# google-research/tnco

Hardware: AMD Instinct MI355X
Metric: SA move-evaluations/s (whole node) + best log10(flops) vs ref, 512-leaf TN (higher is better)
Workload: dtype f64

## Files before the change

tnco_amd/csrc/sa_kernels.h:

```cpp
#pragma once
#include <hip/hip_runtime.h>
#include <stdint.h>

namespace tnco {

#ifndef TNCO_LPS
#define TNCO_LPS 1
#endif
constexpr int LPS = TNCO_LPS;

struct __attribute__((aligned(32))) NodeRec {
  int32_t left, right, parent, pad;
  union { double ccost; double pleft; };
  union { double partial; double pright; };
};
struct __attribute__((aligned(16))) Links {
  int32_t left, right, parent, pad;
};
struct __attribute__((aligned(128))) ReplicaState {
  double min_cost;
  double init_total;
  unsigned long long n_moves, n_accepted, n_improved;
  int32_t mti;
  int32_t mtw;
  int32_t status;
  int32_t jinvalid;
  unsigned long long n_randpick;
  uint32_t jmin, jtail;
  double total;
  unsigned long long n_fullcopy;
  unsigned long long pad1[5];
};
static_assert(sizeof(NodeRec) == 32, "NodeRec");
static_assert(sizeof(ReplicaState) == 128, "ReplicaState");

struct Params {
  int32_t n, N, I, W;
  int32_t BS;
  int32_t WS;
  int32_t WOFF;
  int64_t RB;
  int32_t jcap;
  int64_t R;
  uint8_t* blocks;
  int32_t* lpar;
  uint32_t* mt;
  uint32_t* mtshadow;
  ReplicaState* rs;
  Links* minlinks;
  int32_t* jlog;
  const uint64_t* leafmask;
  const uint64_t* outmask;
  int32_t cost_mode;
  int32_t log2d;
  const double* ctab;
  const double* dimsd;
  const uint64_t* oddmask;
  int32_t odd_single;
  const uint64_t* sparse;
  double n_projs;
  int32_t f32;
  int32_t disable_shared;
  const uint64_t* dimclass;
  int32_t n_dimclass;
  int32_t cpl;
};

template <int K>
struct Mask {
  uint64_t w[K];
};
template <int K>
__device__ __forceinline__ Mask<K> mzero() {
  Mask<K> r;
#pragma unroll
  for (int k = 0; k < K; ++k) r.w[k] = 0;
  return r;
}
#define TNCO_MASK_OP(NAME, EXPR)                                                  \
  template <int K>                                                                \
  __device__ __forceinline__ Mask<K> NAME(const Mask<K>& a, const Mask<K>& b) {   \
    Mask<K> r;                                                                    \
    _Pragma("unroll") for (int k = 0; k < K; ++k) r.w[k] = (EXPR);                \
    return r;                                                                     \
  }
TNCO_MASK_OP(mand, a.w[k] & b.w[k])
TNCO_MASK_OP(mor, a.w[k] | b.w[k])
TNCO_MASK_OP(mxor, a.w[k] ^ b.w[k])
TNCO_MASK_OP(mandn, a.w[k] & ~b.w[k])
#undef TNCO_MASK_OP
template <int K>
__device__ __forceinline__ uint32_t mpopc(const Mask<K>& a) {
  uint32_t c = 0;
#pragma unroll
  for (int k = 0; k < K; ++k) c += (uint32_t)__popcll(a.w[k]);
  return c;
}
template <int K>
__device__ __forceinline__ bool mnonzero(const Mask<K>& a) {
  uint64_t x = 0;
#pragma unroll
  for (int k = 0; k < K; ++k) x |= a.w[k];
  return x != 0;
}
template <int K>
__device__ __forceinline__ bool mdiffer(const Mask<K>& a, const Mask<K>& b) {
  return mnonzero<K>(mxor<K>(a, b));
}
template <int K>
__device__ __forceinline__ Mask<K> msel(bool c, const Mask<K>& a, const Mask<K>& b) {
  Mask<K> r;
#pragma unroll
  for (int k = 0; k < K; ++k) r.w[k] = c ? a.w[k] : b.w[k];
  return r;
}

typedef uint64_t u64x2 __attribute__((ext_vector_type(2)));
typedef uint32_t u32x2 __attribute__((ext_vector_type(2)));
template <int K>
struct PairStage {
  u64x2 p[K / 2 ? K / 2 : 1];
  uint64_t s;
};
template <int LOG2L, int K, bool HYPER, bool UNI = false, bool PAIRS = false>
struct View {
  static constexpr int L = 1 << LOG2L;
  static constexpr int LK = L * K;
  static constexpr int KP = K / 2;
  uint8_t* blk;
  int32_t* lpar;
  const uint64_t* leafmask;
  uint64_t* hyp;
  int n, BS, W, lig, WS, WOFF;

  __device__ __forceinline__ void init(const Params& P, uint8_t* blk_, int32_t* lpar_, int lig_, uint64_t* hyp_ = nullptr) {
    blk = blk_; lpar = lpar_; leafmask = P.leafmask; n = P.n; BS = P.BS; W = P.W; lig = lig_;
    WS = P.WS; WOFF = P.WOFF; hyp = hyp_;
  }
  __device__ __forceinline__ NodeRec* hdr(int p) const {
    return reinterpret_cast<NodeRec*>(blk + (int64_t)(p - n) * BS);
  }
  __device__ __forceinline__ uint32_t hdr_piece_off(int p) const { return (uint32_t)(p - n) * (uint32_t)BS + 8u * (uint32_t)(lig & 3); }
  __device__ __forceinline__ int widx(int k) const {
    if constexpr (PAIRS) return k < 2 * KP ? 2 * L * (k >> 1) + 2 * lig + (k & 1) : 2 * L * KP + lig;
    return k * L + lig;
  }
  __device__ __forceinline__ uint64_t* words(int p) const {
    if constexpr (UNI) return reinterpret_cast<uint64_t*>(blk + (int64_t)(p - n) * BS + 32);
    return reinterpret_cast<uint64_t*>(blk + WOFF + (int64_t)(p - n) * WS);
  }
  __device__ __forceinline__ uint64_t* hwords(int p) const { return hyp + (int64_t)(p - n) * W; }
  __device__ __forceinline__ Mask<K> mask(int x) const {
    const bool leaf = x < n;
    const uint64_t* s = leaf ? leafmask + (int64_t)x * LK : words(x);
    Mask<K> r;
#pragma unroll
    for (int k = 0; k < K; ++k) {
      const int i = widx(k);
      r.w[k] = s[(leaf || i < W) ? i : W - 1];
    }
#pragma unroll
    for (int k = 0; k < K; ++k)
      if (!leaf && widx(k) >= W) r.w[k] = 0ull;
    return r;
  }
  __device__ __forceinline__ Mask<K> mask_staged(int x) const {
    const bool leaf = x < n;
    const uint64_t* s = leaf ? leafmask + (int64_t)x * LK : words(x);
    Mask<K> r;
#pragma unroll
    for (int k = 0; k < K; ++k) {
      r.w[k] = 0ull;
      if (leaf || widx(k) < W) r.w[k] = s[widx(k)];
    }
    return r;
  }
  __device__ __forceinline__ void mask_stage_into(Mask<K>& r, int x) const {
    const bool leaf = x < n;
    const uint64_t* s = leaf ? leafmask + (int64_t)x * LK : words(x);
#pragma unroll
    for (int k = 0; k < K; ++k)
      if (leaf || widx(k) < W) r.w[k] = s[widx(k)];
  }
  __device__ __forceinline__ void set_mask(int p, const Mask<K>& v) const {
    uint64_t* s = words(p);
#pragma unroll
    for (int k = 0; k < K; ++k)
      if (widx(k) < W) s[widx(k)] = v.w[k];
  }
  __device__ __forceinline__ void pair_stage_into(PairStage<K>& g, int x) const {
    const bool leaf = x < n;
    const uint64_t* s = leaf ? leafmask + (int64_t)x * LK : words(x);
#pragma unroll
    for (int j = 0; j < KP; ++j)
      if (leaf || widx(2 * j) < W) g.p[j] = *reinterpret_cast<const u64x2*>(s + widx(2 * j));
    if constexpr (K & 1)
      if (leaf || widx(K - 1) < W) g.s = s[widx(K - 1)];
  }
  __device__ __forceinline__ Mask<K> pair_landed(PairStage<K>& g) const {
    Mask<K> r;
#pragma unroll
    for (int j = 0; j < KP; ++j) {
      if (widx(2 * j + 1) >= W) g.p[j].y = 0ull;
      r.w[2 * j] = g.p[j].x;
      r.w[2 * j + 1] = g.p[j].y;
    }
    if constexpr (K & 1) r.w[K - 1] = g.s;
    return r;
  }
  __device__ __forceinline__ void set_mask_pairs(int p, const Mask<K>& v) const {
    uint64_t* s = words(p);
#pragma unroll
    for (int j = 0; j < KP; ++j)
      if (widx(2 * j) < W) {
        u64x2 t;
        t.x = v.w[2 * j]; t.y = v.w[2 * j + 1];
        *reinterpret_cast<u64x2*>(s + widx(2 * j)) = t;
      }
    if constexpr (K & 1)
      if (widx(K - 1) < W) s[widx(K - 1)] = v.w[K - 1];
  }
  __device__ __forceinline__ void set_mask_first(int p, const Mask<K>& v) const {
    if (widx(0) < W) words(p)[widx(0)] = v.w[0];
  }
  __device__ __forceinline__ Mask<K> hyper(int p) const {
    Mask<K> r = mzero<K>();
    if constexpr (HYPER) {
      const uint64_t* s = hwords(p);
#pragma unroll
      for (int k = 0; k < K; ++k)
        if (widx(k) < W) r.w[k] = s[widx(k)];
    }
    return r;
  }
  __device__ __forceinline__ void set_hyper(int p, const Mask<K>& v) const {
    if constexpr (HYPER) {
      if (hyp == nullptr) return;
      uint64_t* s = hwords(p);
#pragma unroll
      for (int k = 0; k < K; ++k)
        if (widx(k) < W) s[widx(k)] = v.w[k];
    }
  }
  __device__ __forceinline__ double partial(int x) const {
    const double* a = x < n ? reinterpret_cast<const double*>(leafmask) : &hdr(x)->partial;
    const double p = *a;
    return x < n ? 0.0 : p;
  }
  __device__ __forceinline__ int parent(int x) const {
    const int32_t* a = x < n ? lpar + (int64_t)x * LPS : &hdr(x)->parent;
    return *a;
  }
  __device__ __forceinline__ void set_parent(int x, int p) const {
    if (x < n) lpar[(int64_t)x * LPS] = p; else hdr(x)->parent = p;
  }
  __device__ __forceinline__ void set_parent_group(int x, int p) const {
    if (x < n) {
      if constexpr (LPS == 16) {
        if (lig < 4) *reinterpret_cast<int4*>(lpar + (int64_t)x * LPS + 4 * lig) = make_int4(p, p, p, p);
      } else {
        if (lig == 0) lpar[(int64_t)x * LPS] = p;
      }
    } else if (lig == 0) {
      hdr(x)->parent = p;
    }
  }
  __device__ __forceinline__ void set_parent_lane0(int x, int p) const {
    int32_t* a = x < n ? lpar + (int64_t)x * LPS : &hdr(x)->parent;
    if (lig == 0) *a = p;
  }
  __device__ __forceinline__ int left(int x) const { return x < n ? -1 : hdr(x)->left; }
  __device__ __forceinline__ int right(int x) const { return x < n ? -1 : hdr(x)->right; }
};

__device__ inline int cpl_cost_exp(const Params& P, const uint8_t* blk, int lk, int l, int rr) {
  auto legs = [&](int x) -> const uint64_t* {
    return x < P.n ? P.leafmask + (int64_t)x * lk : reinterpret_cast<const uint64_t*>(blk + (int64_t)(x - P.n) * P.BS + 32);
  };
  const uint64_t *a = legs(l), *b = legs(rr);
  int pc = 0;
  for (int w = 0; w < P.W; ++w) pc += __popcll(a[w] | b[w]);
  return P.log2d * pc;
}
__device__ inline double cpl_partial(const Params& P, const uint8_t* blk, int64_t r, int p, int parent) {
  if (parent < 0) return P.rs[r].total;
  const NodeRec* h = reinterpret_cast<const NodeRec*>(blk + (int64_t)(parent - P.n) * P.BS);
  return h->left == p ? h->pleft : h->pright;
}

#define TNCO_DPP_XOR1 0xB1
#define TNCO_DPP_XOR2 0x4E
#define TNCO_DPP_HALF_MIRROR 0x141
#define TNCO_DPP_MIRROR 0x140

template <int CTRL>
__device__ __forceinline__ uint32_t dpp(uint32_t v) {
  return (uint32_t)__builtin_amdgcn_update_dpp(0, (int)v, CTRL, 0xF, 0xF, false);
}

template <int J>
__device__ __forceinline__ uint32_t quad_bcast(uint32_t v) {
  return dpp<J * 0x55>(v);
}

template <int LOG2L>
__device__ __forceinline__ uint32_t gsum(uint32_t v) {
  if constexpr (LOG2L >= 1) v += dpp<TNCO_DPP_XOR1>(v);
  if constexpr (LOG2L >= 2) v += dpp<TNCO_DPP_XOR2>(v);
  if constexpr (LOG2L >= 3) v += dpp<TNCO_DPP_HALF_MIRROR>(v);
  if constexpr (LOG2L >= 4) v += dpp<TNCO_DPP_MIRROR>(v);
  if constexpr (LOG2L >= 5) v += (uint32_t)__shfl_xor((int)v, 16);
  if constexpr (LOG2L >= 6) v += (uint32_t)__shfl_xor((int)v, 32);
  return v;
}

template <int LOG2L>
__device__ __forceinline__ uint32_t gmax(uint32_t v) {
  auto mx = [](uint32_t a, uint32_t b) { return a > b ? a : b; };
  if constexpr (LOG2L >= 1) v = mx(v, dpp<TNCO_DPP_XOR1>(v));
  if constexpr (LOG2L >= 2) v = mx(v, dpp<TNCO_DPP_XOR2>(v));
  if constexpr (LOG2L >= 3) v = mx(v, dpp<TNCO_DPP_HALF_MIRROR>(v));
  if constexpr (LOG2L >= 4) v = mx(v, dpp<TNCO_DPP_MIRROR>(v));
  if constexpr (LOG2L >= 5) v = mx(v, (uint32_t)__shfl_xor((int)v, 16));
  if constexpr (LOG2L >= 6) v = mx(v, (uint32_t)__shfl_xor((int)v, 32));
  return v;
}

template <int LOG2L>
__device__ __forceinline__ bool gany(bool p) {
  return gsum<LOG2L>(p ? 1u : 0u) != 0u;
}

__device__ __forceinline__ double rnd_cost(double x, int f32) {
  return f32 ? (double)(float)x : x;
}

__device__ __forceinline__ double pow2_cost(int e, int f32) {
  double v = (e > 1023) ? __builtin_huge_val() : __hiloint2double((1023 + e) << 20, 0);
  return f32 ? (double)(float)v : v;
}

typedef __attribute__((address_space(3))) const double lds_cdouble;

template <int LOG2L>
__device__ __forceinline__ uint64_t group_bcast(uint64_t x, int j, int gbase) {
  uint32_t lo = (uint32_t)x, hi = (uint32_t)(x >> 32);
  if constexpr (LOG2L <= 2) {
    uint32_t l2, h2;
    switch (j) {
      case 0: l2 = dpp<0x00>(lo); h2 = dpp<0x00>(hi); break;
      case 1: l2 = dpp<0x55>(lo); h2 = dpp<0x55>(hi); break;
      case 2: l2 = dpp<0xAA>(lo); h2 = dpp<0xAA>(hi); break;
// ... 393 lines not shown
```

tnco_amd/csrc/sa_sweep.h:

```cpp
#pragma once
#include "sa_kernels.h"
#include "fw_params.h"

#include <type_traits>

namespace tnco {

#define TNCO_LANDED(x) __asm__ volatile("" : "+v"(x) : : "memory")

#ifndef TNCO_NODE_ACCESS
#define TNCO_NODE_ACCESS 4
#endif

#define TNCO_LDS __attribute__((address_space(3)))
typedef TNCO_LDS volatile uint32_t lds_vu32;
typedef TNCO_LDS volatile int32_t lds_vi32;

__device__ __forceinline__ uint32_t mt_temper(uint32_t z) {
  z ^= (z >> 11);
  z ^= (z << 7) & 0x9d2c5680u;
  z ^= (z << 15) & 0xefc60000u;
  z ^= (z >> 18);
  return z;
}

constexpr int MT_SHADOW = 64;

constexpr int MT_ROUND_RING = 64;
constexpr int MT_ROUND_LOW = 8;
static_assert(MT_ROUND_RING <= MT_SHADOW && MT_ROUND_LOW >= 7, "refill rounds");

typedef uint32_t rng_u32x4 __attribute__((ext_vector_type(4)));
struct RngPcv { rng_u32x4 pcv; };
struct RngNoPcv {};
template <int LOG2L, int RINGX = 0, bool PCV = false>
struct Rng : std::conditional_t<PCV, RngPcv, RngNoPcv> {
  static constexpr int L = 1 << LOG2L;
  static constexpr int NL = L < 4 ? L : 4;
  static constexpr int SB = 4 * NL;
  static constexpr int RING = RINGX ? RINGX : ((2 * SB > 16) ? 2 * SB : 16);
  static_assert(RING <= MT_SHADOW && (RING & (RING - 1)) == 0 && RING >= 2 * SB, "ring size");

  struct __attribute__((packed, aligned(4))) U4 { uint32_t x[4]; };

  uint32_t* mt_base;
  uint32_t* sh_base;
  uint32_t r32;
  lds_vu32* ring;
  int lig;
  __device__ __forceinline__ uint32_t* st() const { return mt_base + (uint64_t)r32 * 624u; }
  __device__ __forceinline__ uint32_t* shadow() const { return sh_base + (uint64_t)r32 * (uint32_t)MT_SHADOW; }
  uint32_t cons, prod, tw;
  bool pend, ptw;
  typedef rng_u32x4 u32x4;
  u32x4 pa;
  uint32_t pb, pc[4];
  typedef u32x4 u32x4w __attribute__((aligned(4)));

  __device__ __forceinline__ uint32_t gen_of_cons() const { return cons == 0 ? 0u : (cons - 1u) / 624u; }

  __device__ __forceinline__ void request() {
    const uint32_t k0 = prod % 624u;
    ptw = prod >= tw;
    if (lig < NL) {
      const int k = (int)k0 + 4 * lig;
      const uint32_t* s = st();
      pa = *reinterpret_cast<const u32x4*>(s + k);
      if (ptw) {
        pb = s[(k + 4 == 624) ? 0 : k + 4];
        if (k == 224) {
          if constexpr (PCV) { this->pcv.x = s[621]; this->pcv.y = s[622]; this->pcv.z = s[623]; this->pcv.w = s[0]; }
          else { pc[0] = s[621]; pc[1] = s[622]; pc[2] = s[623]; pc[3] = s[0]; }
        } else {
          int km = k + 397;
          if (km >= 624) km -= 624;
          if constexpr (PCV) {
            this->pcv = *reinterpret_cast<const u32x4w*>(s + km);
          } else {
            const U4 c = *reinterpret_cast<const U4*>(s + km);
            pc[0] = c.x[0]; pc[1] = c.x[1]; pc[2] = c.x[2]; pc[3] = c.x[3];
          }
        }
      }
    }
    pend = true;
  }
  __device__ __forceinline__ void produce() {
    if (lig < NL) {
      const uint32_t nx[4] = {pa[1], pa[2], pa[3], pb};
      uint32_t v[4];
#pragma unroll
      for (int j = 0; j < 4; ++j) {
        v[j] = pa[j];
        if (ptw) {
// ... 144 lines not shown
  } while (0)
#define TNCO_PROF_OUT(rs) \
  for (int k_ = 0; k_ < 5; ++k_) (rs)->pad1[k_] += pa_[k_]
#else
#define TNCO_PROF_DECL
#define TNCO_PROF_T(i)
#define TNCO_PROF_F(i)
#define TNCO_PROF_ACC
#define TNCO_PROF_OUT(rs)
#endif

#ifndef TNCO_SWEEP_THREADS
#define TNCO_SWEEP_THREADS 256
#endif
constexpr int SWT = TNCO_SWEEP_THREADS;
#ifndef TNCO_FW_STAGED_WAVES
#define TNCO_FW_STAGED_WAVES 2
#endif
#ifndef TNCO_LEAN_RULE
#define TNCO_LEAN_RULE (FW && !GENERIC && !HYPER && LOG2L == 2)
#endif
template <int LOG2L, int K, bool HYPER, bool GENERIC, bool FW = false, bool SPREAD = false>
#ifndef TNCO_HYPER_WAVES
#define TNCO_HYPER_WAVES 2
#endif
#ifndef TNCO_GENERIC_WAVES
#define TNCO_GENERIC_WAVES 2
#endif
#ifndef TNCO_K4_WAVES
#define TNCO_K4_WAVES 2
#endif
__device__ __forceinline__ void sa_run_body(
    const Params& P, const double* __restrict__ betas, const int64_t n_steps, const int prob_kind,
    const FwParams& F, const int tail_last, const int block0) {
  constexpr int L = 1 << LOG2L;
  constexpr int GPB = SWT >> LOG2L;
  using M = Mask<K>;
  constexpr bool ROUNDS = !HYPER && !GENERIC && !FW;
  constexpr bool RPCV = ROUNDS && TNCO_NODE_ACCESS >= 4;
  using R = Rng<LOG2L, ROUNDS ? MT_ROUND_RING : 0, RPCV>;
  static_assert(!ROUNDS || R::SB + 1 >= MT_ROUND_LOW, "refill rounds: the prologue");
  __shared__ uint32_t rngbuf[GPB * R::RING];
  __shared__ ColdState coldbuf[GPB];
  __shared__ int32_t jbuf[GPB * 16];
  constexpr bool LEAN = TNCO_LEAN_RULE;
  __shared__ WalkScal scalbuf[LEAN ? GPB : 1];
  __shared__ uint64_t slbuf[LEAN && FW ? GPB * L * K : 1];
  __shared__ double tabbuf[GENERIC ? (L * K * 64 + 1) : 1];
  __shared__ uint64_t clsbuf[GENERIC ? (TABS_MAXCLS * L * K) : 1];
  __shared__ uint64_t oddbuf[GENERIC ? (L * K) : 1];
  if constexpr (GENERIC) {
    const bool use_ctab = P.cost_mode == 1 || (P.cost_mode == 2 && P.odd_single);
    if (use_ctab) {
      for (int i = threadIdx.x; i < P.W * 64 + 1; i += SWT) tabbuf[i] = P.ctab[i];
    } else if (P.cost_mode == 2) {
      for (int i = threadIdx.x; i < L * K * 64; i += SWT) tabbuf[i] = P.dimsd[i];
    }
    if (P.cost_mode >= 2) {
      for (int i = threadIdx.x; i < P.n_dimclass * L * K; i += SWT) clsbuf[i] = P.dimclass[i];
      if (P.cost_mode == 2)
        for (int i = threadIdx.x; i < L * K; i += SWT) oddbuf[i] = P.oddmask[i];
    }
    __syncthreads();
  }

  const int tid = threadIdx.x;
  const int lig = tid & (L - 1);
  const int gbase = (tid & 63) & ~(L - 1);
  const int seats = SPREAD ? block0 : (64 >> LOG2L);
  const int gw = (tid & 63) >> LOG2L;
  const bool master = !SPREAD || gw < seats;
  const int seat = SPREAD ? (gw & (seats - 1)) : gw;
  const int gib = SPREAD ? (tid >> 6) * (64 >> LOG2L) + seat : tid >> LOG2L;
  const int64_t r = SPREAD ? ((int64_t)blockIdx.x * (SWT / 64) + (tid >> 6)) * seats + seat
                           : ((int64_t)blockIdx.x + block0) * GPB + gib;
  if (r >= P.R || n_steps <= 0) return;
  const bool lane0 = (lig == 0) && master;
  const int slig = master ? lig : (1 << 20);

  const int n = P.n, N = P.N;
  constexpr bool HYD = HYPER;
  constexpr bool CP = !HYPER && !GENERIC && !FW;
  constexpr bool QHDR = CP && TNCO_NODE_ACCESS >= 1, PAIRS = CP && TNCO_NODE_ACCESS >= 2, PSEL = CP && TNCO_NODE_ACCESS >= 3 && LPS == 1;
  View<LOG2L, K, HYPER, !FW, PAIRS> v;
  v.init(P, P.blocks + r * P.RB, nullptr, lig);
  auto lpar = [&]() -> int32_t* { return P.lpar + r * (int64_t)n * LPS; };
  lds_cold& cold = *((lds_cold*)coldbuf + gib);

  R rng;
  {
    const ReplicaState* rs = P.rs + r;
    rng.template init<ROUNDS ? 2 : 0>(P, r, (lds_vu32*)rngbuf + gib * R::RING, rs->mti, rs->mtw, master ? lig : 64);
    if (lane0) {
      cold.min_cost = rs->min_cost;
      cold.jmin = rs->jmin;
      cold.n_impr = 0; cold.n_full = 0; cold.n_rpick = 0;
    }
  }
  const uint32_t jcap = (uint32_t)P.jcap;
  uint32_t jtail = P.rs[r].jtail;
  bool jinvalid = P.rs[r].jinvalid != 0;
  auto jb = [&](int i) -> lds_vi32& { return *((lds_vi32*)jbuf + gib * 16 + i); };
  auto jlog = [&]() -> int32_t* {
    uint32_t rr = rng.r32;
    __asm__ volatile("" : "+v"(rr));
    return P.jlog + (int64_t)rr * (int64_t)P.jcap;
  };
  if ((jtail & 15u) != 0u) {
    for (int q = slig; q < 4; q += L) {
      const int4 t = *reinterpret_cast<const int4*>(jlog() + (jtail & ~15u) + 4 * q);
      jb(4 * q + 0) = t.x; jb(4 * q + 1) = t.y; jb(4 * q + 2) = t.z; jb(4 * q + 3) = t.w;
    }
  }
  M sl_regs = mzero<K>();
  typedef TNCO_LDS volatile uint64_t lds_vu64;
  [[maybe_unused]] lds_vu64* slw = (lds_vu64*)slbuf + (LEAN && FW ? gib * (L * K) : 0);
  [[maybe_unused]] bool impr_any = false;
  if constexpr (FW) {
    const uint64_t* s0 = F.slices + r * 2 * (int64_t)(L * K);
#pragma unroll
    for (int k = 0; k < K; ++k) {
      if constexpr (LEAN && FW) slw[v.widx(k)] = s0[v.widx(k)]; else sl_regs.w[k] = s0[v.widx(k)];
    }
  }
  [[maybe_unused]] TabsLds<K> tabs{P, (lds_cdouble*)tabbuf, (lds_cu64*)clsbuf, (lds_cu64*)oddbuf, mzero<K>()};
  if constexpr (GENERIC) {
    if (P.sparse != nullptr) {
#pragma unroll
      for (int k = 0; k < K; ++k) tabs.sp.w[k] = P.sparse[k * L + lig];
    }
  }
  const int f32 = GENERIC ? P.f32 : 0;
  const int log2d = P.log2d;
  const bool disable_shared = P.disable_shared != 0;
  const int nsteps32 = (int)n_steps;

  int B = 0, bl = 0, br = 0, A = -1;
  [[maybe_unused]] int wB = 0;
  double ccB = 0, partB = 0;
  WalkScal scal_regs{0, 0, 0, 0, 0, 0, 0, -1, -1, -1, -1, -1, -1, 0, 0, 0, 0};
  TNCO_LDS volatile WalkScal* scal_lds = (TNCO_LDS volatile WalkScal*)scalbuf + (LEAN ? gib : 0);
  auto& S = *[&]() {
    if constexpr (LEAN) return scal_lds; else return &scal_regs;
  }();
  if constexpr (CP) {
    double t0 = P.rs[r].total;
    TNCO_LANDED(t0);
    S.total = t0;
  }
  if constexpr (LEAN) {
    S.total = 0; S.beta = 0; S.pP = 0; S.pO = 0; S.pC = 0; S.raC = 0; S.rnC = 0;
    S.raL = -1; S.raR = -1; S.raP = -1; S.rnL = -1; S.rnR = -1; S.rnP = -1; S.raW = 0; S.rnW = 0; S.n_moves = 0; S.n_acc = 0;
  }
  M mP = mzero<K>(), mO = mzero<K>(), hB = mzero<K>();
  bool pl = true;
  M mC = mzero<K>(), hA = mzero<K>();
  int step = 0;
  int state = S_BEGIN;

  int stC = 0, stE = 0;
  [[maybe_unused]] double stW64 = 0;
  [[maybe_unused]] double stQ0 = 0, stQ1 = 0;
  int x_al = 0, x_ar = 0, x_aP = -1;
  double x_ccA = 0, x_partA = 0, x_pCcur = 0;
  int gL = -1, gR = -1, gP = -1;
  [[maybe_unused]] int gW = 0;
  double gC = 0;
  [[maybe_unused]] double gQ1 = 0;
  typedef int32_t i32x4 __attribute__((ext_vector_type(4)));
  [[maybe_unused]] i32x4 gLRP = (i32x4)(-1);
  [[maybe_unused]] u32x2 gHq = (u32x2)(0u);
  M gM = mzero<K>(), gH = mzero<K>();
  [[maybe_unused]] PairStage<K> gMq;
  if constexpr (PAIRS) {
#pragma unroll
    for (int j = 0; j < (K / 2 ? K / 2 : 1); ++j) gMq.p[j] = (u64x2)(0ull);
    gMq.s = 0ull;
  }
  uint32_t gXlo = 0, gXhi = 0;

  TNCO_PROF_DECL;
  for (;;) {
    TNCO_PROF_T(0);
    if (rng.pend) rng.produce();
    TNCO_PROF_T(1);

    bool acc = false, did_move = false, did_end = false, improved = false;

    if (state == S_END) {
      did_end = true;
      const bool close_sweep = !FW || tail_last != 0 || step != nsteps32 - 1;
      if constexpr (CP) {
        stQ0 = pl ? S.pP : S.pO;
        stQ1 = pl ? S.pO : S.pP;
      }
      if (close_sweep && partB < cold.min_cost) {
        if constexpr (FW) impr_any = true;
        if (lane0) {
          cold.min_cost = partB;
          cold.n_impr = cold.n_impr + 1;
        }
        if (jinvalid) {
          if (lane0) {
            NodeRec o;
            o.left = bl; o.right = br; o.parent = -1; o.pad = 0; o.ccost = CP ? stQ0 : ccB; o.partial = CP ? stQ1 : partB;
            *v.hdr(B) = o;
          }
          v.lpar = lpar();
          Links* __restrict__ ml = P.minlinks + r * (int64_t)N;
          for (int i0 = slig; i0 < N; i0 += 4 * L) {
            int4 h4[4];
#pragma unroll
            for (int q = 0; q < 4; ++q) {
              const int i = i0 + q * L;
              h4[q] = make_int4(-1, -1, -1, 0);
              if (i < n) h4[q].z = v.lpar[(int64_t)i * LPS];
              else if (i < N) h4[q] = *reinterpret_cast<const int4*>(v.hdr(i));
            }
#pragma unroll
            for (int q = 0; q < 4; ++q) {
              const int i = i0 + q * L;
              if (i < N) {
                Links o;
                o.left = h4[q].x; o.right = h4[q].y; o.parent = h4[q].z; o.pad = 0;
                ml[i] = o;
              }
            }
          }
          jtail = 0;
          jinvalid = false;
          if (lane0) cold.n_full = cold.n_full + 1;
        }
        improved = true;
      }
      if constexpr (CP) S.total = partB;
      ++step;
      state = (step >= nsteps32) ? -1 : S_BEGIN;
    }

    TNCO_PROF_F(1);
    int hN = -1, x1 = -1, yN = -1;
    const uint32_t* xa = nullptr;
    if (state == S_BEGIN) {
      const uint32_t x = rng.next();
      x_al = (int)(x % (uint32_t)n);
      x1 = x_al;
      xa = reinterpret_cast<const uint32_t*>(lpar() + (int64_t)x_al * LPS);
    } else if (state == S_GOT_B) {
      hN = B;
      if constexpr (CP) x1 = B;
      else xa = reinterpret_cast<const uint32_t*>(&v.hdr(B)->partial);
    } else if (CP && state == S_GOT_HB) {
      xa = reinterpret_cast<const uint32_t*>(betas + step);
      if (A >= 0) {
        hN = A;
        x1 = A;
      }
    } else if (state == S_GOT_HB) {
      x1 = pl ? br : bl;
      hN = A;
      yN = B;
      xa = reinterpret_cast<const uint32_t*>(&v.hdr(N - 1)->partial);
    } else if (state == S_GOT_B1) {
      xa = reinterpret_cast<const uint32_t*>(betas + step);
      if (A >= 0) {
        hN = S.raP;
        yN = A;
        x1 = (S.raL == B) ? S.raR : S.raL;
      }
    } else if (state == S_MOVE) {
      if constexpr (CP) {
        if (S.raP >= 0) {
          hN = S.raP;
          x1 = S.raP;
        }
      } else if (S.raP >= 0) {
        x1 = (S.rnL == A) ? S.rnR : S.rnL;
        hN = S.rnP;
        yN = S.raP;
      }
    }

    TNCO_PROF_F(2);
    if constexpr (QHDR) {
      int lq = lig;
      __asm__ volatile("" : "+v"(lq));
      v.lig = lq;
    }
    if (hN >= 0) {
      const NodeRec* q = v.hdr(hN);
      if constexpr (QHDR) {
        gHq = *reinterpret_cast<const u32x2*>(v.blk + v.hdr_piece_off(hN));
      } else {
        if constexpr (CP) gLRP = *reinterpret_cast<const i32x4*>(q);
        else { gL = q->left; gR = q->right; gP = q->parent; }
        gC = q->ccost;
        if constexpr (FW) gW = q->pad;
        if constexpr (CP) gQ1 = q->pright;
      }
    }
    double gMp = 0;
    if (x1 >= 0) {
      if constexpr (PAIRS) v.pair_stage_into(gMq, x1);
      else v.mask_stage_into(gM, x1);
      if constexpr (!CP)
        if (x1 >= n) gMp = v.hdr(x1)->partial;
    }
    if (xa != nullptr) {
      gXlo = xa[0];
      gXhi = xa[1];
    }
    if constexpr (HYPER) {
      if (yN >= 0) v.mask_stage_into(gH, yN);
    }
    if constexpr (ROUNDS) {
      const bool need = !rng.pend && rng.avail() < (uint32_t)MT_ROUND_LOW;
      const bool round = __ballot(need) != 0;
      if (round && rng.room()) rng.request();
    } else {
      if (rng.room()) rng.request();
    }
    TNCO_PROF_F(3);

    if (state == S_MOVE) {
      did_move = true;
      int al = S.raL, ar = S.raR;
      const int aP = S.raP;
      double ccA = S.raC;
      const bool c_is_right = (al == B);
      const int C = c_is_right ? ar : al;

      const M hy = HYD ? mand<K>(hB, mor<K>(mand<K>(hA, mC), mand<K>(mP, mO))) : mzero<K>();
      M sl = sl_regs;
      if constexpr (LEAN && FW) {
#pragma unroll
        for (int k = 0; k < K; ++k) sl.w[k] = slw[v.widx(k)];
      }
      constexpr bool PICK_FIRST = !GENERIC && FW;
      bool interP, interO;
      int pcAP = 0, pcBP = 0, pcAO = 0, pcBO = 0;
      if constexpr (!GENERIC && !PICK_FIRST) {
        uint32_t wP = mpopc<K>(mor<K>(mor<K>(mor<K>(mxor<K>(mP, mC), hy), mO), sl)) |
                      (mpopc<K>(mor<K>(mor<K>(mP, mC), sl)) << 13) | ((mnonzero<K>(mand<K>(mP, mC)) ? 1u : 0u) << 26);
        uint32_t wO = mpopc<K>(mor<K>(mor<K>(mor<K>(mxor<K>(mO, mC), hy), mP), sl)) |
                      (mpopc<K>(mor<K>(mor<K>(mO, mC), sl)) << 13) | ((mnonzero<K>(mand<K>(mO, mC)) ? 1u : 0u) << 26);
        wP = gsum<LOG2L>(wP);
        wO = gsum<LOG2L>(wO);
        interP = (wP >> 26) != 0;
        interO = (wO >> 26) != 0;
        pcAP = (int)(wP & 0x1fffu); pcBP = (int)((wP >> 13) & 0x1fffu);
        pcAO = (int)(wO & 0x1fffu); pcBO = (int)((wO >> 13) & 0x1fffu);
      } else {
        const uint32_t w = gsum<LOG2L>((mnonzero<K>(mand<K>(mP, mC)) ? 1u : 0u) |
                                       ((mnonzero<K>(mand<K>(mO, mC)) ? 1u : 0u) << 8));
        interP = (w & 0xffu) != 0;
        interO = (w >> 8) != 0;
      }
      bool pick0;
      if (disable_shared || (interP && interO)) {
        pick0 = (rng.next() & 1u) != 0;
        if (lane0) cold.n_rpick = cold.n_rpick + 1;
      } else {
        pick0 = pl ? interP : interO;
      }
      const bool pickP = pick0 == pl;
      const M mD = msel<K>(pickP, mP, mO), mE = msel<K>(pickP, mO, mP);
      const M newB = mor<K>(mxor<K>(mD, mC), hy);
      const double pD = pickP ? S.pP : S.pO, pE = pickP ? S.pO : S.pP;
      const int E = pick0 ? br : bl;
      if constexpr (PICK_FIRST) {
        const uint32_t w = gsum<LOG2L>(mpopc<K>(mor<K>(mor<K>(newB, mE), sl)) | (mpopc<K>(mor<K>(mor<K>(mD, mC), sl)) << 13));
        pcAP = pcAO = (int)(w & 0x1fffu);
        pcBP = pcBO = (int)((w >> 13) & 0x1fffu);
      }

      [[maybe_unused]] double new_width_B = 0;
      bool fits = true;
      if constexpr (FW) {
        double sliced_width;
        if constexpr (!GENERIC) {
          const uint32_t x = gsum<LOG2L>(mpopc<K>(newB) | (mpopc<K>(mandn<K>(newB, sl)) << 16));
          new_width_B = (double)(log2d * (int)(x & 0xffffu));
          sliced_width = (double)(log2d * (int)(x >> 16));
        } else if (F.log2dims == nullptr && P.sparse == nullptr) {
          const uint32_t x = gsum<LOG2L>(mpopc<K>(newB) | (mpopc<K>(mandn<K>(newB, sl)) << 16));
          new_width_B = fw_wr(F, F.log2d * (double)(x & 0xffffu));
          sliced_width = fw_wr(F, F.log2d * (double)(x >> 16));
        } else {
          new_width_B = fw_width<LOG2L, K>(P, F, newB, lig, gbase);
          sliced_width = fw_width<LOG2L, K>(P, F, mandn<K>(newB, sl), lig, gbase);
        }
        fits = sliced_width <= F.max_width;
      }
      double nA, nB;
      if constexpr (!GENERIC) {
        nA = pow2_cost(log2d * (pickP ? pcAP : pcAO), 0);
        nB = pow2_cost(log2d * (pickP ? pcBP : pcBO), 0);
      } else {
        nA = generic_cost_t<LOG2L, K>(P, tabs, mor<K>(mor<K>(newB, mE), sl), lig, gbase);
        nB = generic_cost_t<LOG2L, K>(P, tabs, mor<K>(mor<K>(mD, mC), sl), lig, gbase);
      }
      const double delta = rnd_cost(rnd_cost(nB - ccB, f32) + rnd_cost(nA - ccA, f32), f32);
      ++S.n_moves;

      if (fits) {
        const double u = rng.uniform01();
        acc = accept_move(prob_kind, S.beta, delta, S.total, u, f32);
      }

      double pEcur = pE, pCcur = S.pC;
      M mBnow, mX;
      stC = C; stE = E;
      if (acc) {
        ++S.n_acc;
        if constexpr (FW) {
          if (F.width_f32) wB = __float_as_int((float)new_width_B);
          stW64 = new_width_B;
        }
        if (pick0) br = C; else bl = C;
        if (c_is_right) ar = E; else al = E;
        if constexpr (HYD) hB = newB;
        ccB = nB;
        ccA = nA;
        S.total = rnd_cost(S.total + delta, f32);
        pEcur = S.pC;
        pCcur = pE;
        mBnow = newB;
        mX = mE;
      } else {
        mBnow = HYD ? hB : mxor<K>(mP, mO);
        mX = mC;
      }
      if constexpr (CP) {
        stQ0 = pick0 ? pD : pEcur;
        stQ1 = pick0 ? pEcur : pD;
      }
      partB = rnd_cost(rnd_cost(pD + pEcur, f32) + ccB, f32);
      const double partA = rnd_cost(rnd_cost(partB + pCcur, f32) + ccA, f32);
      x_al = al; x_ar = ar; x_aP = aP; x_ccA = ccA; x_partA = partA; x_pCcur = pCcur;
      mP = mBnow; mO = mX; pl = c_is_right;
    }

    TNCO_PROF_T(2);
    if constexpr (QHDR) {
      TNCO_LANDED(gHq);
    } else {
      TNCO_LANDED(gL); TNCO_LANDED(gR); TNCO_LANDED(gP); TNCO_LANDED(gC);
      if constexpr (CP) { TNCO_LANDED(gQ1); TNCO_LANDED(gLRP); }
    }
    if constexpr (FW) TNCO_LANDED(gW);
    TNCO_LANDED(gMp); TNCO_LANDED(gXlo); TNCO_LANDED(gXhi);
    if constexpr (PAIRS) {
#pragma unroll
      for (int j = 0; j < K / 2; ++j) TNCO_LANDED(gMq.p[j]);
      if constexpr (K & 1) TNCO_LANDED(gMq.s);
    } else {
#pragma unroll
      for (int k = 0; k < K; ++k) {
        TNCO_LANDED(gM.w[k]);
        if constexpr (HYPER) { TNCO_LANDED(gH.w[k]); }
      }
    }
    TNCO_LANDED(rng.pb);
    TNCO_LANDED(rng.pa);
#pragma unroll
    for (int j = 0; j < 4; ++j) TNCO_LANDED(rng.pc[j]);
    if constexpr (RPCV) TNCO_LANDED(rng.pcv);

    TNCO_PROF_T(3);
    if constexpr (QHDR) {
      int lq = lig;
      __asm__ volatile("" : "+v"(lq));
      v.lig = lq;
    }
    if (did_move && acc) {
      if (!jinvalid) {
        if (jtail == jcap) {
          jinvalid = true;
        } else {
          if (lane0) jb((int)(jtail & 15u)) = stE;
          ++jtail;
          if ((jtail & 15u) == 0u) {
            for (int q = slig; q < 4; q += L)
              *reinterpret_cast<int4*>(jlog() + (jtail - 16u) + 4 * q) =
                  make_int4(jb(4 * q + 0), jb(4 * q + 1), jb(4 * q + 2), jb(4 * q + 3));
          }
        }
      }
      v.lpar = lpar();
      if (master) {
        if constexpr (PSEL) {
          v.set_parent_lane0(stC, B);
          v.set_parent_lane0(stE, A);
        } else {
          v.set_parent_group(stC, B);
          v.set_parent_group(stE, A);
        }
        if constexpr (PAIRS) v.set_mask_pairs(B, mP);
        else v.set_mask(B, mP);
      }
    }
    if (did_move || did_end) {
      if constexpr (QHDR) {
        if (master && v.lig < 4) {
          const uint64_t q0 = __double_as_longlong(stQ0), q1 = __double_as_longlong(stQ1);
          u32x2 o;
          const int lq = v.lig;
          o.x = lq == 0 ? (uint32_t)bl : (lq == 1 ? (uint32_t)A : (uint32_t)(lq == 2 ? q0 : q1));
          o.y = lq == 0 ? (uint32_t)br : (lq == 1 ? 0u : (uint32_t)((lq == 2 ? q0 : q1) >> 32));
          *reinterpret_cast<u32x2*>(v.blk + v.hdr_piece_off(B)) = o;
        }
      } else if (lane0) {
        NodeRec o;
        o.left = bl; o.right = br; o.parent = A; o.pad = FW ? wB : 0;
        if constexpr (CP) { o.pleft = stQ0; o.pright = stQ1; } else { o.ccost = ccB; o.partial = partB; }
        *v.hdr(B) = o;
        if constexpr (FW) {
          if (did_move && acc && !F.width_f32) F.width64[(int64_t)rng.r32 * N + B] = stW64;
        }
      }
#ifdef TNCO_FIRST64
      if (!(did_move && acc))
        v.set_mask_first(B, did_move ? mP : (HYD ? hB : mxor<K>(mP, mO)));
#endif
      if (improved && lane0) cold.jmin = jtail;
      if (state < 0) break;
    }
    TNCO_PROF_T(4);
    TNCO_PROF_ACC;

    if constexpr (QHDR) {
      gL = (int)quad_bcast<0>(gHq.x); gR = (int)quad_bcast<0>(gHq.y); gP = (int)quad_bcast<1>(gHq.x);
      gC = __hiloint2double((int)quad_bcast<2>(gHq.y), (int)quad_bcast<2>(gHq.x));
      gQ1 = __hiloint2double((int)quad_bcast<3>(gHq.y), (int)quad_bcast<3>(gHq.x));
    } else if constexpr (CP) { gL = gLRP.x; gR = gLRP.y; gP = gLRP.z; }
    if constexpr (PAIRS) gM = v.pair_landed(gMq);
    auto land_A = [&]() {
      S.raL = gL; S.raR = gR; S.raP = gP;
      const M mB = mxor<K>(mP, mO);
      mC = mxor<K>(gM, mB);
      S.pC = (gL == B) ? gQ1 : gC;
      S.raC = pow2_cost(log2d * (int)gsum<LOG2L>(mpopc<K>(mor<K>(mB, gM))), 0);
    };
    if (CP && did_move) {
      S.pP = partB; S.pO = x_pCcur;
      B = A; bl = x_al; br = x_ar; ccB = x_ccA; partB = x_partA;
      A = x_aP;
      if (A >= 0) land_A();
      state = (A < 0) ? S_END : S_MOVE;
    } else if (CP && state == S_GOT_B) {
      bl = gL; br = gR; A = gP;
      pl = gL == x_al;
      mO = mxor<K>(gM, mP);
      S.pO = pl ? gQ1 : gC;
      partB = S.total;
      ccB = pow2_cost(log2d * (int)gsum<LOG2L>(mpopc<K>(mor<K>(mP, mO))), 0);
      state = S_GOT_HB;
    } else if (CP && state == S_GOT_HB) {
      S.beta = __hiloint2double((int)gXhi, (int)gXlo);
      if (A >= 0) land_A();
      state = (A < 0) ? S_END : S_MOVE;
    } else if (did_move) {
      S.pP = partB; S.pO = x_pCcur;
      B = A; bl = x_al; br = x_ar; ccB = x_ccA; partB = x_partA;
      if constexpr (HYPER) { hB = hA; hA = gH; }
      A = x_aP;
      S.raL = S.rnL; S.raR = S.rnR; S.raP = S.rnP; S.raC = S.rnC;
      S.rnL = gL; S.rnR = gR; S.rnP = gP; S.rnC = gC;
      if constexpr (FW) { wB = S.raW; S.raW = S.rnW; S.rnW = gW; }
      mC = gM;
      S.pC = gMp;
      state = (A < 0) ? S_END : S_MOVE;
    } else if (state == S_BEGIN) {
      B = (int)gXlo;
      mP = gM; S.pP = CP ? 0.0 : gMp;
      state = S_GOT_B;
    } else if (state == S_GOT_B) {
      bl = gL; br = gR; A = gP; ccB = gC;
      if constexpr (FW) wB = gW;
      partB = __hiloint2double((int)gXhi, (int)gXlo);
      pl = gL == x_al;
      state = S_GOT_HB;
    } else if (state == S_GOT_HB) {
      mO = gM; S.pO = gMp;
      S.total = __hiloint2double((int)gXhi, (int)gXlo);
      S.raL = gL; S.raR = gR; S.raP = gP; S.raC = gC;
      if constexpr (FW) S.raW = gW;
      if constexpr (HYPER) { hB = gH; }
      state = S_GOT_B1;
    } else if (state == S_GOT_B1) {
      mC = gM; S.pC = gMp;
      S.beta = __hiloint2double((int)gXhi, (int)gXlo);
      S.rnL = gL; S.rnR = gR; S.rnP = gP; S.rnC = gC;
      if constexpr (FW) S.rnW = gW;
      if constexpr (HYPER) { hA = gH; }
      state = (A < 0) ? S_END : S_MOVE;
    }
  }

  if ((jtail & 15u) != 0u) {
    for (int q = slig; q < 4; q += L)
      *reinterpret_cast<int4*>(jlog() + (jtail & ~15u) + 4 * q) =
          make_int4(jb(4 * q + 0), jb(4 * q + 1), jb(4 * q + 2), jb(4 * q + 3));
  }
  if constexpr (FW) {
    if (impr_any) {
      uint64_t* s1 = F.slices + r * 2 * (int64_t)(L * K) + L * K;
#pragma unroll
      for (int k = 0; k < K; ++k)
        if (master) s1[v.widx(k)] = (LEAN && FW) ? (uint64_t)slw[v.widx(k)] : sl_regs.w[k];
    }
  }
  int mti, mtw;
  rng.finish(mti, mtw);
  if (lane0) {
    ReplicaState* rs = P.rs + r;
    if constexpr (CP) rs->total = S.total;
    rs->jmin = cold.jmin; rs->jtail = jtail;
    rs->jinvalid = jinvalid ? 1 : 0;
// ... 33 lines not shown
```

Before: 11.66 billion.

## Pack node header and leg masks into one contiguous line per node

Adds a node-line layout for the 4-lane, 3-word case: the header fields and the leg-mask words of a node now sit in adjacent 16-byte chunks, so each lane makes one 16-byte load and one pair load per node visit instead of separate header and mask loads. Lanes 0-1 hold the header, and the missing first mask word is passed between lanes with a DPP swizzle. Accepted moves write both parent pointers in one lane-parallel store instead of two lane-0 stores. The default node access level goes from 4 to 6, so this path is active for supported shapes. In exchange there is extra cross-lane shuffling and select logic, and the leaf-mask addressing uses a negative bias trick.

Measured after the change: 12.92 billion, median of 4. +10.8%, better.

```diff
diff --git a/tnco_amd/csrc/node_line.h b/tnco_amd/csrc/node_line.h
--- /dev/null
+++ b/tnco_amd/csrc/node_line.h
@@ -0,0 +1,41 @@
+#pragma once
+
+namespace tnco {
+namespace node_line {
+
+constexpr int CHUNK = 16;
+constexpr int HDR_CHUNKS = 2;
+constexpr int ACCESSES = 2;
+
+constexpr bool supported(int L, int K) { return L == 4 && K == 3; }
+
+constexpr int chunk(int L, int r, int j) { return r * L + j; }
+constexpr int byte_off(int L, int r, int j) { return CHUNK * chunk(L, r, j); }
+constexpr int leg_word(int c) { return 2 * (c - HDR_CHUNKS); }
+constexpr int chunk_word(int c) { return c < HDR_CHUNKS ? -1 : leg_word(c); }
+
+constexpr int LEAF_BIAS = CHUNK * HDR_CHUNKS;
+
+constexpr bool reads(int L, int r, int j, int W, bool leaf) {
+  return leaf ? chunk_word(chunk(L, r, j)) >= 0 : chunk_word(chunk(L, r, j)) < W;
+}
+
+constexpr bool gives(int L, int j) { return chunk(L, 0, j) >= HDR_CHUNKS; }
+constexpr int taker(int j) { return j ^ 2; }
+constexpr bool takes(int L, int j) { return !gives(L, j); }
+constexpr int handed_word(int L, int j) { return leg_word(chunk(L, 0, j)) + 1; }
+
+constexpr int slot_word(int L, int , int j, int k) {
+  return k == 0 ? (gives(L, j) ? leg_word(chunk(L, 0, j)) : handed_word(L, taker(j)))
+                : leg_word(chunk(L, 1, j)) + (k - 1);
+}
+
+struct Src {
+  int lane, slot;
+};
+constexpr Src store_src(int L, int r, int j, int h) {
+  return r == 0 ? (h == 0 ? Src{j, 0} : Src{taker(j), 0}) : Src{j, 1 + h};
+}
+
+}
+}
diff --git a/tnco_amd/csrc/sa_kernels.h b/tnco_amd/csrc/sa_kernels.h
--- a/tnco_amd/csrc/sa_kernels.h
+++ b/tnco_amd/csrc/sa_kernels.h
@@ -1,6 +1,8 @@
 #pragma once
 #include <hip/hip_runtime.h>
 #include <stdint.h>
+
+#include "node_line.h"
 
 namespace tnco {
 
@@ -122,8 +124,16 @@
   u64x2 p[K / 2 ? K / 2 : 1];
   uint64_t s;
 };
-template <int LOG2L, int K, bool HYPER, bool UNI = false, bool PAIRS = false>
+template <int CTRL>
+__device__ __forceinline__ uint32_t dpp(uint32_t v);
+typedef uint32_t u32x4 __attribute__((ext_vector_type(4)));
+struct LineStage {
+  u32x4 a;
+  u64x2 b;
+};
+template <int LOG2L, int K, bool HYPER, bool UNI = false, bool PAIRS = false, bool LINE = false>
 struct View {
+  static_assert(!LINE || (PAIRS && UNI && node_line::supported(1 << LOG2L, K)), "the chunk map: 4 lanes x 3 words");
   static constexpr int L = 1 << LOG2L;
   static constexpr int LK = L * K;
   static constexpr int KP = K / 2;
@@ -142,6 +152,7 @@
   }
   __device__ __forceinline__ uint32_t hdr_piece_off(int p) const { return (uint32_t)(p - n) * (uint32_t)BS + 8u * (uint32_t)(lig & 3); }
   __device__ __forceinline__ int widx(int k) const {
+    if constexpr (LINE) return node_line::slot_word(L, K, lig, k);
     if constexpr (PAIRS) return k < 2 * KP ? 2 * L * (k >> 1) + 2 * lig + (k & 1) : 2 * L * KP + lig;
     return k * L + lig;
   }
@@ -219,6 +230,46 @@
       }
     if constexpr (K & 1)
       if (widx(K - 1) < W) s[widx(K - 1)] = v.w[K - 1];
+  }
+  __device__ __forceinline__ void line_stage_into(LineStage& g, int x) const {
+    const bool leaf = x < n;
+    const uint8_t* s = leaf ? reinterpret_cast<const uint8_t*>(leafmask) : blk;
+    const uint32_t o = (leaf ? (uint32_t)x * (uint32_t)(8 * LK) - (uint32_t)node_line::LEAF_BIAS : (uint32_t)(x - n) * (uint32_t)BS) +
+                       (uint32_t)node_line::CHUNK * (uint32_t)lig;
+    if (__builtin_expect(!leaf || node_line::gives(L, lig), 1)) g.a = *reinterpret_cast<const u32x4*>(s + o);
+    if (leaf || widx(1) < W) g.b = *reinterpret_cast<const u64x2*>(s + (o + (uint32_t)node_line::byte_off(L, 1, 0)));
+  }
+  __device__ __forceinline__ Mask<K> line_landed(LineStage& g) const {
+    const uint32_t tl = dpp<0x4E>(g.a.z), th = dpp<0x4E>(g.a.w);
+    const bool give = node_line::gives(L, lig);
+    if (widx(1) >= W) g.b.x = 0ull;
+    if (widx(2) >= W) g.b.y = 0ull;
+    Mask<K> r;
+    r.w[0] = ((uint64_t)(give ? g.a.y : th) << 32) | (give ? g.a.x : tl);
+    r.w[1] = g.b.x;
+    r.w[2] = g.b.y;
+    return r;
+  }
+  __device__ __forceinline__ void set_line_row0(int p, int left, int right, int parent, double q0, double q1, const Mask<K>& v,
+                                                bool on, bool legs) const {
+    const uint32_t tl = dpp<0x4E>((uint32_t)v.w[0]), th = dpp<0x4E>((uint32_t)(v.w[0] >> 32));
+    const uint64_t b0 = __double_as_longlong(q0), b1 = __double_as_longlong(q1);
+    const int lq = lig;
+    u32x4 o;
+    o.x = lq == 0 ? (uint32_t)left : (lq == 1 ? (uint32_t)b0 : (uint32_t)v.w[0]);
+    o.y = lq == 0 ? (uint32_t)right : (lq == 1 ? (uint32_t)(b0 >> 32) : (uint32_t)(v.w[0] >> 32));
+    o.z = lq == 0 ? (uint32_t)parent : (lq == 1 ? (uint32_t)b1 : tl);
+    o.w = lq == 0 ? 0u : (lq == 1 ? (uint32_t)(b1 >> 32) : th);
+    if (on && (legs || !node_line::gives(L, lq)))
+      *reinterpret_cast<u32x4*>(blk + ((uint32_t)(p - n) * (uint32_t)BS + (uint32_t)node_line::CHUNK * (uint32_t)lq)) = o;
+  }
+  __device__ __forceinline__ void set_line_row1(int p, const Mask<K>& v) const {
+    if (widx(1) < W) {
+      u64x2 t;
+      t.x = v.w[1]; t.y = v.w[2];
+      *reinterpret_cast<u64x2*>(blk + ((uint32_t)(p - n) * (uint32_t)BS + (uint32_t)node_line::byte_off(L, 1, 0) +
+                                       (uint32_t)node_line::CHUNK * (uint32_t)lig)) = t;
+    }
   }
   __device__ __forceinline__ void set_mask_first(int p, const Mask<K>& v) const {
     if (widx(0) < W) words(p)[widx(0)] = v.w[0];
@@ -268,6 +319,11 @@
   __device__ __forceinline__ void set_parent_lane0(int x, int p) const {
     int32_t* a = x < n ? lpar + (int64_t)x * LPS : &hdr(x)->parent;
     if (lig == 0) *a = p;
+  }
+  __device__ __forceinline__ void set_parent_pair(int xc, int pc, int xe, int pe) const {
+    const int x = lig == 0 ? xc : xe;
+    int32_t* a = x < n ? lpar + (int64_t)x * LPS : &hdr(x)->parent;
+    if (lig < 2) *a = lig == 0 ? pc : pe;
   }
   __device__ __forceinline__ int left(int x) const { return x < n ? -1 : hdr(x)->left; }
   __device__ __forceinline__ int right(int x) const { return x < n ? -1 : hdr(x)->right; }
diff --git a/tnco_amd/csrc/sa_sweep.h b/tnco_amd/csrc/sa_sweep.h
--- a/tnco_amd/csrc/sa_sweep.h
+++ b/tnco_amd/csrc/sa_sweep.h
@@ -9,7 +9,7 @@
 #define TNCO_LANDED(x) __asm__ volatile("" : "+v"(x) : : "memory")
 
 #ifndef TNCO_NODE_ACCESS
-#define TNCO_NODE_ACCESS 4
+#define TNCO_NODE_ACCESS 6
 #endif
 
 #define TNCO_LDS __attribute__((address_space(3)))
@@ -320,7 +320,9 @@
   constexpr bool HYD = HYPER;
   constexpr bool CP = !HYPER && !GENERIC && !FW;
   constexpr bool QHDR = CP && TNCO_NODE_ACCESS >= 1, PAIRS = CP && TNCO_NODE_ACCESS >= 2, PSEL = CP && TNCO_NODE_ACCESS >= 3 && LPS == 1;
-  View<LOG2L, K, HYPER, !FW, PAIRS> v;
+  constexpr bool LINE = CP && TNCO_NODE_ACCESS >= 5 && node_line::supported(L, K);
+  constexpr bool PPAIR = LINE && PSEL && TNCO_NODE_ACCESS >= 6, ROW0 = LINE && TNCO_NODE_ACCESS >= 7;
+  View<LOG2L, K, HYPER, !FW, PAIRS, LINE> v;
   v.init(P, P.blocks + r * P.RB, nullptr, lig);
   auto lpar = [&]() -> int32_t* { return P.lpar + r * (int64_t)n * LPS; };
   lds_cold& cold = *((lds_cold*)coldbuf + gib);
@@ -415,6 +417,8 @@
     for (int j = 0; j < (K / 2 ? K / 2 : 1); ++j) gMq.p[j] = (u64x2)(0ull);
     gMq.s = 0ull;
   }
+  [[maybe_unused]] LineStage gLn;
+  if constexpr (LINE) { gLn.a = (u32x4)(0u); gLn.b = (u64x2)(0ull); }
   uint32_t gXlo = 0, gXhi = 0;
 
   TNCO_PROF_DECL;
@@ -525,7 +529,7 @@
       __asm__ volatile("" : "+v"(lq));
       v.lig = lq;
     }
-    if (hN >= 0) {
+    if (!LINE && hN >= 0) {
       const NodeRec* q = v.hdr(hN);
       if constexpr (QHDR) {
         gHq = *reinterpret_cast<const u32x2*>(v.blk + v.hdr_piece_off(hN));
@@ -539,7 +543,8 @@
     }
     double gMp = 0;
     if (x1 >= 0) {
-      if constexpr (PAIRS) v.pair_stage_into(gMq, x1);
+      if constexpr (LINE) v.line_stage_into(gLn, x1);
+      else if constexpr (PAIRS) v.pair_stage_into(gMq, x1);
       else v.mask_stage_into(gM, x1);
       if constexpr (!CP)
         if (x1 >= n) gMp = v.hdr(x1)->partial;
@@ -680,7 +685,9 @@
     }
 
     TNCO_PROF_T(2);
-    if constexpr (QHDR) {
+    if constexpr (LINE) {
+      TNCO_LANDED(gLn.a); TNCO_LANDED(gLn.b);
+    } else if constexpr (QHDR) {
       TNCO_LANDED(gHq);
     } else {
       TNCO_LANDED(gL); TNCO_LANDED(gR); TNCO_LANDED(gP); TNCO_LANDED(gC);
@@ -688,7 +695,8 @@
     }
     if constexpr (FW) TNCO_LANDED(gW);
     TNCO_LANDED(gMp); TNCO_LANDED(gXlo); TNCO_LANDED(gXhi);
-    if constexpr (PAIRS) {
+    if constexpr (LINE) {
+    } else if constexpr (PAIRS) {
 #pragma unroll
       for (int j = 0; j < K / 2; ++j) TNCO_LANDED(gMq.p[j]);
       if constexpr (K & 1) TNCO_LANDED(gMq.s);
@@ -701,9 +709,12 @@
     }
     TNCO_LANDED(rng.pb);
     TNCO_LANDED(rng.pa);
-#pragma unroll
-    for (int j = 0; j < 4; ++j) TNCO_LANDED(rng.pc[j]);
-    if constexpr (RPCV) TNCO_LANDED(rng.pcv);
+    if constexpr (RPCV) {
+      TNCO_LANDED(rng.pcv);
+    } else {
+#pragma unroll
+      for (int j = 0; j < 4; ++j) TNCO_LANDED(rng.pc[j]);
+    }
 
     TNCO_PROF_T(3);
     if constexpr (QHDR) {
@@ -727,19 +738,24 @@
       }
       v.lpar = lpar();
       if (master) {
-        if constexpr (PSEL) {
+        if constexpr (PPAIR) {
+          v.set_parent_pair(stC, B, stE, A);
+        } else if constexpr (PSEL) {
           v.set_parent_lane0(stC, B);
           v.set_parent_lane0(stE, A);
         } else {
           v.set_parent_group(stC, B);
           v.set_parent_group(stE, A);
         }
-        if constexpr (PAIRS) v.set_mask_pairs(B, mP);
+        if constexpr (LINE) v.set_line_row1(B, mP);
+        else if constexpr (PAIRS) v.set_mask_pairs(B, mP);
         else v.set_mask(B, mP);
       }
     }
     if (did_move || did_end) {
-      if constexpr (QHDR) {
+      if constexpr (LINE) {
+        v.set_line_row0(B, bl, br, A, stQ0, stQ1, mP, master, did_move && (ROW0 || acc));
+      } else if constexpr (QHDR) {
         if (master && v.lig < 4) {
           const uint64_t q0 = __double_as_longlong(stQ0), q1 = __double_as_longlong(stQ1);
           u32x2 o;
@@ -767,12 +783,17 @@
     TNCO_PROF_T(4);
     TNCO_PROF_ACC;
 
-    if constexpr (QHDR) {
+    if constexpr (LINE) {
+      gL = (int)quad_bcast<0>(gLn.a.x); gR = (int)quad_bcast<0>(gLn.a.y); gP = (int)quad_bcast<0>(gLn.a.z);
+      gC = __hiloint2double((int)quad_bcast<1>(gLn.a.y), (int)quad_bcast<1>(gLn.a.x));
+      gQ1 = __hiloint2double((int)quad_bcast<1>(gLn.a.w), (int)quad_bcast<1>(gLn.a.z));
+      gM = v.line_landed(gLn);
+    } else if constexpr (QHDR) {
       gL = (int)quad_bcast<0>(gHq.x); gR = (int)quad_bcast<0>(gHq.y); gP = (int)quad_bcast<1>(gHq.x);
       gC = __hiloint2double((int)quad_bcast<2>(gHq.y), (int)quad_bcast<2>(gHq.x));
       gQ1 = __hiloint2double((int)quad_bcast<3>(gHq.y), (int)quad_bcast<3>(gHq.x));
     } else if constexpr (CP) { gL = gLRP.x; gR = gLRP.y; gP = gLRP.z; }
-    if constexpr (PAIRS) gM = v.pair_landed(gMq);
+    if constexpr (PAIRS && !LINE) gM = v.pair_landed(gMq);
     auto land_A = [&]() {
       S.raL = gL; S.raR = gR; S.raP = gP;
       const M mB = mxor<K>(mP, mO);
```
